# huzi96/gaussian-pcloud-render

Measured on AMD Instinct MI355X. Metric: rendered frames/sec at 1080p (fwd+bwd), THuman-800K, higher is better.
Workload: dtype f32

## Files before the change

gaussian-pcloud-render_amd/csrc/sort.hip:

```cpp
#include "common.hpp"

namespace gsr {

__device__ __forceinline__ uint32_t lane_id() { return __builtin_amdgcn_mbcnt_hi(~0u, __builtin_amdgcn_mbcnt_lo(~0u, 0u)); }

__device__ __forceinline__ uint32_t wave_inclusive_scan(uint32_t v, uint32_t lane)
{
#pragma unroll
    for (int d = 1; d < 64; d <<= 1) {
        const uint32_t n = __shfl_up(v, d, 64);
        if (lane >= (uint32_t)d) v += n;
    }
    return v;
}

__device__ __forceinline__ uint32_t block_exclusive_scan_256(uint32_t v, uint32_t* tmp, uint32_t* total)
{
    const uint32_t lane = threadIdx.x & 63, w = threadIdx.x >> 6;
    const uint32_t inc = wave_inclusive_scan(v, lane);
    if (lane == 63) tmp[w] = inc;
    __syncthreads();
    uint32_t base = 0;
#pragma unroll
    for (int i = 0; i < 4; i++)
        if ((uint32_t)i < w) base += tmp[i];
    if (total) *total = tmp[0] + tmp[1] + tmp[2] + tmp[3];
    __syncthreads();
    return base + inc - v;
}

struct SortView {
    size_t stride;
    const uint64_t* n_dev;
    size_t n_stride;
    int64_t cap;
    const uint32_t* ctl;
};
__device__ __forceinline__ bool pass_control(const SortView& sv, uint32_t view, int shift, uint32_t& base)
{
    base = 0u;
    if (sv.ctl == nullptr) return true;
    const uint32_t* c = at_view(sv.ctl, sv.stride, view);
    base = c[SORTCTL_BASE];
    return (uint32_t)shift < c[SORTCTL_BITS];
}
__device__ __forceinline__ int64_t view_count(const SortView& sv, uint32_t view)
{
    if (sv.n_dev == nullptr) return sv.cap;
    const uint64_t n = *at_view(sv.n_dev, sv.n_stride, view);
    return n < (uint64_t)sv.cap ? (int64_t)n : sv.cap;
}

constexpr int HIST_GROUP = 16;

template <typename KeyT, int RS_ITEMS>
__global__ __launch_bounds__(RS_THREADS) void k_radix_hist(const KeyT* __restrict__ keys, SortView sv, int shift,
                                                           uint32_t mask, uint32_t* __restrict__ hist, int nblk_pad,
                                                           uint32_t* __restrict__ minmax)
{
    constexpr int RS_TILE = RS_THREADS * RS_ITEMS;
    const uint32_t view = blockIdx.y;
    uint32_t kbase;
    if (!pass_control(sv, view, shift, kbase)) return;
    const int64_t n = view_count(sv, view);
    keys = at_view(keys, sv.stride, view);
    hist = at_view(hist, sv.stride, view);
    if (minmax) minmax = at_view(minmax, sv.stride, view);
    const uint32_t d = threadIdx.x;
    if ((int64_t)blockIdx.x * RS_TILE >= n) {
        if (d <= mask) hist[(size_t)d * nblk_pad + blockIdx.x] = 0;
        if (minmax && d == 0) { minmax[blockIdx.x] = 0xFFFFFFFFu; minmax[nblk_pad + blockIdx.x] = 0u; }
        return;
    }
    constexpr int HIST_COPIES = 4 * RS_WAVES;
    __shared__ __attribute__((aligned(16))) uint32_t h[HIST_COPIES][RADIX];
    __shared__ uint32_t s_min, s_max;
    for (int i = threadIdx.x; i < HIST_COPIES * RADIX / 4; i += RS_THREADS) reinterpret_cast<uint4*>(&h[0][0])[i] = make_uint4(0, 0, 0, 0);
    if (threadIdx.x == 0) { s_min = 0xFFFFFFFFu; s_max = 0u; }
    __syncthreads();
    uint32_t kmin = 0xFFFFFFFFu, kmax = 0u;
    const int64_t base = (int64_t)blockIdx.x * RS_TILE;
    const uint32_t w = (threadIdx.x >> 6) * 4u + (threadIdx.x & 3u);
    if (sizeof(KeyT) == 2 && RS_ITEMS % 8 == 0 && base + RS_TILE <= n) {
        const uint4* k4 = reinterpret_cast<const uint4*>(keys + base) + threadIdx.x * (RS_ITEMS / 8);
#pragma unroll
        for (int v = 0; v < RS_ITEMS / 8; v++) {
            const uint4 q = k4[v];
            const uint32_t wds[4] = {q.x, q.y, q.z, q.w};
#pragma unroll
            for (int j = 0; j < 4; j++) {
                atomicAdd(&h[w][((wds[j] & 0xFFFFu) >> shift) & mask], 1u);
                atomicAdd(&h[w][((wds[j] >> 16) >> shift) & mask], 1u);
            }
        }
    } else {
#pragma unroll
        for (int i = 0; i < RS_ITEMS; i++) {
            const int64_t idx = base + i * RS_THREADS + threadIdx.x;
            if (idx < n) {
                const uint32_t key = (uint32_t)keys[idx];
                atomicAdd(&h[w][((key - kbase) >> shift) & mask], 1u);
                if (key != CULLED_KEY) { kmin = key < kmin ? key : kmin; kmax = key > kmax ? key : kmax; }
            }
        }
    }
    if (minmax) {
#pragma unroll
        for (int dd = 32; dd >= 1; dd >>= 1) {
            const uint32_t a = __shfl_xor(kmin, dd, 64), b = __shfl_xor(kmax, dd, 64);
            kmin = a < kmin ? a : kmin;
            kmax = b > kmax ? b : kmax;
        }
        if ((threadIdx.x & 63) == 0) { atomicMin(&s_min, kmin); atomicMax(&s_max, kmax); }
    }
    __syncthreads();
    if (minmax && d == 0) { minmax[blockIdx.x] = s_min; minmax[nblk_pad + blockIdx.x] = s_max; }
    if (d <= mask) {
        uint32_t c = 0;
#pragma unroll
        for (int i = 0; i < HIST_COPIES; i++) c += h[i][d];
        hist[(size_t)d * nblk_pad + blockIdx.x] = c;
    }
}

__global__ __launch_bounds__(256) void k_radix_rowscan(uint32_t* __restrict__ hist, uint32_t* __restrict__ totals, int nblk_pad,
                                                       size_t stride, const uint32_t* __restrict__ ctl, int shift,
                                                       const uint32_t* __restrict__ minmax, uint32_t* __restrict__ ctl_out,
                                                       uint32_t nrows)
{
    __shared__ uint32_t tmp[4];
    if (blockIdx.x == nrows) {
        minmax = at_view(minmax, stride, blockIdx.y);
        uint32_t kmin = 0xFFFFFFFFu, kmax = 0u;
        for (int b = threadIdx.x; b < nblk_pad; b += 256) {
            const uint32_t a = minmax[b], c = minmax[nblk_pad + b];
            kmin = a < kmin ? a : kmin;
            kmax = c > kmax ? c : kmax;
        }
        __shared__ uint32_t s_min, s_max;
        if (threadIdx.x == 0) { s_min = 0xFFFFFFFFu; s_max = 0u; }
        __syncthreads();
        atomicMin(&s_min, kmin);
        atomicMax(&s_max, kmax);
        __syncthreads();
        if (threadIdx.x == 0) {
            uint32_t* c = at_view(ctl_out, stride, blockIdx.y);
            const uint32_t base = s_min <= s_max ? (s_min & ~(uint32_t)(RADIX - 1)) : 0u;
            const uint32_t span = s_min <= s_max ? s_max - base : 0u;
            const uint32_t bits = span ? 32u - (uint32_t)__builtin_clz(span) : 0u;
            c[SORTCTL_BASE] = base;
            c[SORTCTL_BITS] = bits < (uint32_t)RADIX_BITS ? (uint32_t)RADIX_BITS : bits;
        }
        return;
    }
    if (ctl != nullptr && (uint32_t)shift >= at_view(ctl, stride, blockIdx.y)[SORTCTL_BITS]) return;
    hist = at_view(hist, stride, blockIdx.y);
    totals = at_view(totals, stride, blockIdx.y);
    uint32_t* row = hist + (size_t)blockIdx.x * nblk_pad;
    uint32_t carry = 0;
    for (int b0 = 0; b0 < nblk_pad; b0 += 256) {
        const int b = b0 + threadIdx.x;
        const uint32_t v = b < nblk_pad ? row[b] : 0u;
        uint32_t tot;
        const uint32_t ex = block_exclusive_scan_256(v, tmp, &tot);
        if (b < nblk_pad) row[b] = carry + ex;
        carry += tot;
    }
    if (threadIdx.x == 0) totals[blockIdx.x] = carry;
}

#ifdef GSR_STATS
constexpr int SC_REC = 65536;
__device__ unsigned g_sc_rec[SC_REC][5];
#define SC_T(var) const unsigned long long var = wall_clock64()
#define SC_PUT(i, v) do { if (threadIdx.x == 0) { const unsigned r_ = blockIdx.y * gridDim.x + blockIdx.x; if (r_ < SC_REC) g_sc_rec[r_][i] = (unsigned)(v); } } while (0)
int debug_scatter_times(unsigned long long* out8, int reset)
{
    static unsigned host[SC_REC][5];
    if (hipMemcpyFromSymbol(host, HIP_SYMBOL(g_sc_rec), sizeof(host)) != hipSuccess) return -1;
    for (int i = 0; i < 8; i++) out8[i] = 0;
    for (int r = 0; r < SC_REC; r++) {
        if (host[r][1] == 0) continue;
        for (int i = 0; i < 5; i++) out8[i] += host[r][i];
        out8[5]++;
    }
    if (reset) {
        for (int r = 0; r < SC_REC; r++) for (int i = 0; i < 5; i++) host[r][i] = 0;
        if (hipMemcpyToSymbol(HIP_SYMBOL(g_sc_rec), host, sizeof(host)) != hipSuccess) return -1;
    }
    return 0;
}
#else
#define SC_T(var) do { } while (0)
#define SC_PUT(i, v) do { } while (0)
#endif

template <int BITS, typename KeyT, int RS_ITEMS>
__global__ __launch_bounds__(RS_THREADS) void k_radix_scatter(const KeyT* __restrict__ keys_in,
                                                              const uint32_t* __restrict__ vals_in,
                                                              KeyT* __restrict__ keys_out,
                                                              uint32_t* __restrict__ vals_out, SortView sv, int shift,
                                                              uint32_t mask, const uint32_t* __restrict__ hist,
                                                              const uint32_t* __restrict__ totals, int nblk_pad)
{
    constexpr int RS_TILE = RS_THREADS * RS_ITEMS;
    const uint32_t view = blockIdx.y;
    uint32_t kbase;
    if (!pass_control(sv, view, shift, kbase)) return;
    const int64_t n = view_count(sv, view);
    const uint32_t wg = blockIdx.x, xcd = wg & 7u, r = wg >> 3;
    const uint32_t blk = ((r / HIST_GROUP) * 8u + xcd) * HIST_GROUP + (r % HIST_GROUP);
    hist = at_view(hist, sv.stride, view);
    totals = at_view(totals, sv.stride, view);
    if ((int64_t)blk * RS_TILE >= n) return;
    keys_in = at_view(keys_in, sv.stride, view);
    if (vals_in) vals_in = at_view(vals_in, sv.stride, view);
    keys_out = at_view(keys_out, sv.stride, view);
    vals_out = at_view(vals_out, sv.stride, view);
    __shared__ uint32_t s_key[RS_TILE];
    __shared__ uint32_t s_val[RS_TILE];
    __shared__ uint32_t wave_cnt[RS_WAVES][RADIX];
    __shared__ uint32_t local_base[RADIX];
    __shared__ uint32_t global_base[RADIX];
    __shared__ uint32_t tmp[4];

    const uint32_t tid = threadIdx.x, lane = tid & 63, w = tid >> 6;
    const int64_t blk_base = (int64_t)blk * RS_TILE;
    const int64_t seg_base = blk_base + (int64_t)w * (RS_TILE / RS_WAVES);

    for (int i = lane; i < RADIX; i += 64) wave_cnt[w][i] = 0;
    SC_T(t0);

    const uint32_t tot_d = tid <= mask ? totals[tid] : 0u;
    const uint32_t hist_d = tid <= mask ? hist[(size_t)tid * nblk_pad + blk] : 0u;

    uint32_t k[RS_ITEMS], v[RS_ITEMS], rank[RS_ITEMS];
    const bool full = blk_base + RS_TILE <= n;
    {
        const KeyT* kp = keys_in + seg_base + lane;
        const uint32_t* vp = vals_in ? vals_in + seg_base + lane : nullptr;
        if (full) {
#pragma unroll
            for (int j = 0; j < RS_ITEMS; j++) k[j] = (uint32_t)kp[j * 64] - kbase;
            if (vp) {
#pragma unroll
                for (int j = 0; j < RS_ITEMS; j++) v[j] = vp[j * 64];
            } else {
#pragma unroll
                for (int j = 0; j < RS_ITEMS; j++) v[j] = (uint32_t)(seg_base + j * 64 + lane);
            }
        } else {
#pragma unroll
            for (int j = 0; j < RS_ITEMS; j++) {
                const int64_t idx = seg_base + j * 64 + lane;
                const bool ok = idx < n;
                k[j] = ok ? (uint32_t)kp[j * 64] - kbase : 0xFFFFFFFFu;
                v[j] = ok ? (vp ? vp[j * 64] : (uint32_t)idx) : 0u;
            }
        }
    }
    uint32_t gbase_d = block_exclusive_scan_256(tot_d, tmp, nullptr) + hist_d;
    __builtin_amdgcn_wave_barrier();
#ifdef GSR_STATS
    asm volatile("s_waitcnt vmcnt(0)" ::: "memory");
#endif
    SC_T(t1);
    SC_PUT(0, t1 - t0);

#pragma unroll
    for (int j = 0; j < RS_ITEMS; j++) {
        const bool ok = full || seg_base + j * 64 + lane < n;
        const uint32_t d = (k[j] >> shift) & mask;
        const uint64_t okb = full ? ~0ull : __ballot(ok);
        uint32_t plo = (uint32_t)okb, phi = (uint32_t)(okb >> 32);
#pragma unroll
        for (int b = 0; b < BITS; b++) {
            const uint32_t m = (uint32_t)__builtin_amdgcn_sbfe((int32_t)k[j], (uint32_t)(shift + b), 1u);
            const uint64_t bal = __ballot(m != 0u);
            plo = __builtin_amdgcn_bitop3_b32(plo, (uint32_t)bal, m, 0x90);
            phi = __builtin_amdgcn_bitop3_b32(phi, (uint32_t)(bal >> 32), m, 0x90);
        }
        const uint32_t before = wave_cnt[w][d];
        const uint32_t below = __builtin_amdgcn_mbcnt_hi(phi, __builtin_amdgcn_mbcnt_lo(plo, 0u));
        rank[j] = before + below;
        __builtin_amdgcn_wave_barrier();
        if (ok && below == 0) wave_cnt[w][d] = before + (uint32_t)__popc(plo) + (uint32_t)__popc(phi);
        __builtin_amdgcn_wave_barrier();
    }
    __syncthreads();
    SC_T(t2);
    SC_PUT(1, t2 - t1);

    {
        const uint32_t d = tid;
        uint32_t c[RS_WAVES], run = 0;
#pragma unroll
        for (int i = 0; i < RS_WAVES; i++) {
            c[i] = wave_cnt[i][d];
            wave_cnt[i][d] = run;
            run += c[i];
        }
        const uint32_t lbase = block_exclusive_scan_256(run, tmp, nullptr);
        local_base[d] = lbase;
        global_base[d] = gbase_d;
    }
    __syncthreads();
    SC_T(t3);
    SC_PUT(2, t3 - t2);

#pragma unroll
    for (int j = 0; j < RS_ITEMS; j++) {
        if (full || seg_base + j * 64 + lane < n) {
            const uint32_t d = (k[j] >> shift) & mask;
            const uint32_t pos = local_base[d] + wave_cnt[w][d] + rank[j];
            s_key[pos] = k[j];
            s_val[pos] = v[j];
        }
    }
    __syncthreads();
    SC_T(t4);
    SC_PUT(3, t4 - t3);

    const int64_t rem = n - blk_base;
    const uint32_t count = rem < RS_TILE ? (uint32_t)rem : (uint32_t)RS_TILE;
#pragma unroll
    for (int i = 0; i < RS_ITEMS; i++) {
        const uint32_t p = i * RS_THREADS + tid;
        if (p < count) {
            const uint32_t key = s_key[p];
            const uint32_t d = (key >> shift) & mask;
            const size_t g = (size_t)global_base[d] + (p - local_base[d]);
            keys_out[g] = (KeyT)(key + kbase);
            vals_out[g] = s_val[p];
        }
    }
#ifdef GSR_STATS
    { SC_T(t5); SC_PUT(4, t5 - t4); }
#endif
}

int launch_radix_sort_pairs(const Launch& L, const SortJob& job, bool iota_vals, int end_bit, int* result_buffer, bool key16)
{
    int cur = 0;
    if (job.cap > 0 && job.V > 0) {
        const bool small = job.small_blocks && !key16 && end_bit % RADIX_BITS == 0;
        const int tile = small ? RS_TILE_SMALL : RS_TILE;
        const int nblk = (int)div_up(job.cap, tile);
        const int nblk_pad = sort_hist_stride(job.cap, tile);
        SortView sv{job.stride, job.n_dev, job.n_stride, job.cap, nullptr};
        const dim3 grid_hist(nblk_pad, job.V);
        const dim3 grid((unsigned)div_up(nblk, 8 * HIST_GROUP) * 8 * HIST_GROUP, job.V);
        bool first = true;
        const int npass = (end_bit + RADIX_BITS - 1) / RADIX_BITS;
        int shift = 0;
        for (int pass = 0; pass < npass; pass++) {
            const int bits = (end_bit - shift + (npass - pass) - 1) / (npass - pass);
            const uint32_t mask = (1u << bits) - 1u;
            const bool make_ctl = job.sortctl != nullptr && pass == 0;
            sv.ctl = (job.sortctl != nullptr && pass > 0) ? job.sortctl : nullptr;
            uint32_t* minmax = make_ctl ? job.blk_minmax : nullptr;
            if (key16)
                hipLaunchKernelGGL((k_radix_hist<uint16_t, RS_ITEMS>), grid_hist, dim3(RS_THREADS), 0, L.stream, (const uint16_t*)job.key[cur], sv,
                                   shift, mask, job.hist, nblk_pad, minmax);
            else if (small)
                hipLaunchKernelGGL((k_radix_hist<uint32_t, RS_ITEMS_SMALL>), grid_hist, dim3(RS_THREADS), 0, L.stream, (const uint32_t*)job.key[cur], sv,
                                   shift, mask, job.hist, nblk_pad, minmax);
            else
                hipLaunchKernelGGL((k_radix_hist<uint32_t, RS_ITEMS>), grid_hist, dim3(RS_THREADS), 0, L.stream, (const uint32_t*)job.key[cur], sv,
                                   shift, mask, job.hist, nblk_pad, minmax);
            if (int e = check_launch(L, "radix_hist")) return e;
            hipLaunchKernelGGL(k_radix_rowscan, dim3(mask + 1u + (make_ctl ? 1u : 0u), job.V), dim3(256), 0, L.stream, job.hist,
                               job.totals, nblk_pad, job.stride, sv.ctl, shift, (const uint32_t*)minmax, job.sortctl, mask + 1u);
            if (int e = check_launch(L, "radix_rowscan")) return e;
            const uint32_t* vin = (first && iota_vals) ? (const uint32_t*)nullptr : (const uint32_t*)job.val[cur];
#define GSR_SCATTER(B)                                                                                                        \
    case B:                                                                                                                   \
        if (key16)                                                                                                            \
            hipLaunchKernelGGL((k_radix_scatter<B, uint16_t, RS_ITEMS>), grid, dim3(RS_THREADS), 0, L.stream,                 \
                               (const uint16_t*)job.key[cur], vin, (uint16_t*)job.key[cur ^ 1], job.val[cur ^ 1], sv, shift,  \
                               mask, job.hist, job.totals, nblk_pad);                                                         \
        else                                                                                                                  \
            hipLaunchKernelGGL((k_radix_scatter<B, uint32_t, RS_ITEMS>), grid, dim3(RS_THREADS), 0, L.stream,                 \
                               (const uint32_t*)job.key[cur], vin, job.key[cur ^ 1], job.val[cur ^ 1], sv, shift, mask,       \
                               job.hist, job.totals, nblk_pad);                                                               \
        break;
            if (small)
                hipLaunchKernelGGL((k_radix_scatter<RADIX_BITS, uint32_t, RS_ITEMS_SMALL>), grid, dim3(RS_THREADS), 0, L.stream,
                                   (const uint32_t*)job.key[cur], vin, job.key[cur ^ 1], job.val[cur ^ 1], sv, shift, mask, job.hist,
                                   job.totals, nblk_pad);
            else switch (bits) {
                GSR_SCATTER(1) GSR_SCATTER(2) GSR_SCATTER(3) GSR_SCATTER(4) GSR_SCATTER(5) GSR_SCATTER(6) GSR_SCATTER(7)
                GSR_SCATTER(8)
            }
#undef GSR_SCATTER
            if (int e = check_launch(L, "radix_scatter")) return e;
            cur ^= 1;
            first = false;
            shift += bits;
        }
    } else {
        cur = ((end_bit + RADIX_BITS - 1) / RADIX_BITS) & 1;
    }
    *result_buffer = cur;
    return GSR_OK;
}

}
```

Before: 2153.

## Restructure radix histogram: digit-major copies sized by pass bits, coalesced prefetch

Reworks the radix histogram kernel so the shared-memory histogram is digit-major, with the number of per-thread copies scaled to the pass's digit count (template NB chosen from bits). Keys for full tiles are now loaded with coalesced 16-byte strided loads issued before the shared-memory clear, and the 32-bit key path also uses vector loads. The final reduction reads four uint4s per thread and combines them with a wave shuffle. The aim is fewer atomic conflicts and cheaper reductions on narrow passes, and overlap of global loads with shared init. The cost is more template instantiations and added register pressure from holding keys in registers.

```diff
diff --git a/gaussian-pcloud-render_amd/csrc/sort.hip b/gaussian-pcloud-render_amd/csrc/sort.hip
--- a/gaussian-pcloud-render_amd/csrc/sort.hip
+++ b/gaussian-pcloud-render_amd/csrc/sort.hip
@@ -52,13 +52,19 @@
 }
 
 constexpr int HIST_GROUP = 16;
-
-template <typename KeyT, int RS_ITEMS>
+constexpr int HIST_WORDS = 4 * RS_WAVES * RADIX;
+
+template <typename KeyT, int RS_ITEMS, int NB>
 __global__ __launch_bounds__(RS_THREADS) void k_radix_hist(const KeyT* __restrict__ keys, SortView sv, int shift,
                                                            uint32_t mask, uint32_t* __restrict__ hist, int nblk_pad,
                                                            uint32_t* __restrict__ minmax)
 {
     constexpr int RS_TILE = RS_THREADS * RS_ITEMS;
+    constexpr int NV = RS_ITEMS * (int)sizeof(KeyT) / 16;
+    static_assert(NV >= 1 && NV * 16 == RS_ITEMS * (int)sizeof(KeyT), "a thread's keys of a full block are whole 16-B loads");
+    constexpr uint32_t COPIES = HIST_WORDS / NB;
+    constexpr uint32_t GROUPS = RS_THREADS / NB;
+    static_assert((NB == 64 || NB == 128 || NB == 256) && COPIES == 16 * GROUPS, "a thread sums 16 words");
     const uint32_t view = blockIdx.y;
     uint32_t kbase;
     if (!pass_control(sv, view, shift, kbase)) return;
@@ -72,25 +78,36 @@
         if (minmax && d == 0) { minmax[blockIdx.x] = 0xFFFFFFFFu; minmax[nblk_pad + blockIdx.x] = 0u; }
         return;
     }
-    constexpr int HIST_COPIES = 4 * RS_WAVES;
-    __shared__ __attribute__((aligned(16))) uint32_t h[HIST_COPIES][RADIX];
+    const int64_t base = (int64_t)blockIdx.x * RS_TILE;
+    const bool full = base + RS_TILE <= n;
+    uint4 q[NV];
+    if (full) {
+        const uint4* k4 = reinterpret_cast<const uint4*>(keys + base) + threadIdx.x;
+#pragma unroll
+        for (int v = 0; v < NV; v++) q[v] = k4[v * RS_THREADS];
+    }
+    __shared__ __attribute__((aligned(16))) uint32_t h[HIST_WORDS];
     __shared__ uint32_t s_min, s_max;
-    for (int i = threadIdx.x; i < HIST_COPIES * RADIX / 4; i += RS_THREADS) reinterpret_cast<uint4*>(&h[0][0])[i] = make_uint4(0, 0, 0, 0);
+    for (int i = threadIdx.x; i < HIST_WORDS / 4; i += RS_THREADS) reinterpret_cast<uint4*>(h)[i] = make_uint4(0, 0, 0, 0);
     if (threadIdx.x == 0) { s_min = 0xFFFFFFFFu; s_max = 0u; }
     __syncthreads();
     uint32_t kmin = 0xFFFFFFFFu, kmax = 0u;
-    const int64_t base = (int64_t)blockIdx.x * RS_TILE;
-    const uint32_t w = (threadIdx.x >> 6) * 4u + (threadIdx.x & 3u);
-    if (sizeof(KeyT) == 2 && RS_ITEMS % 8 == 0 && base + RS_TILE <= n) {
-        const uint4* k4 = reinterpret_cast<const uint4*>(keys + base) + threadIdx.x * (RS_ITEMS / 8);
-#pragma unroll
-        for (int v = 0; v < RS_ITEMS / 8; v++) {
-            const uint4 q = k4[v];
-            const uint32_t wds[4] = {q.x, q.y, q.z, q.w};
+    const uint32_t copy = threadIdx.x & (COPIES - 1u);
+    const auto count = [&](uint32_t digit) { atomicAdd(&h[digit * COPIES + copy], 1u); };
+    if (full) {
+#pragma unroll
+        for (int v = 0; v < NV; v++) {
+            const uint32_t wds[4] = {q[v].x, q[v].y, q[v].z, q[v].w};
 #pragma unroll
             for (int j = 0; j < 4; j++) {
-                atomicAdd(&h[w][((wds[j] & 0xFFFFu) >> shift) & mask], 1u);
-                atomicAdd(&h[w][((wds[j] >> 16) >> shift) & mask], 1u);
+                if (sizeof(KeyT) == 2) {
+                    count(((wds[j] & 0xFFFFu) >> shift) & mask);
+                    count(((wds[j] >> 16) >> shift) & mask);
+                } else {
+                    const uint32_t key = wds[j];
+                    count(((key - kbase) >> shift) & mask);
+                    if (key != CULLED_KEY) { kmin = key < kmin ? key : kmin; kmax = key > kmax ? key : kmax; }
+                }
             }
         }
     } else {
@@ -99,7 +116,7 @@
             const int64_t idx = base + i * RS_THREADS + threadIdx.x;
             if (idx < n) {
                 const uint32_t key = (uint32_t)keys[idx];
-                atomicAdd(&h[w][((key - kbase) >> shift) & mask], 1u);
+                count(((key - kbase) >> shift) & mask);
                 if (key != CULLED_KEY) { kmin = key < kmin ? key : kmin; kmax = key > kmax ? key : kmax; }
             }
         }
@@ -115,12 +132,16 @@
     }
     __syncthreads();
     if (minmax && d == 0) { minmax[blockIdx.x] = s_min; minmax[nblk_pad + blockIdx.x] = s_max; }
-    if (d <= mask) {
-        uint32_t c = 0;
-#pragma unroll
-        for (int i = 0; i < HIST_COPIES; i++) c += h[i][d];
-        hist[(size_t)d * nblk_pad + blockIdx.x] = c;
-    }
+    uint32_t c = 0;
+#pragma unroll
+    for (int i = 0; i < 4; i++) {
+        const uint4 x = reinterpret_cast<const uint4*>(h)[d * 4 + i];
+        c += x.x + x.y + x.z + x.w;
+    }
+#pragma unroll
+    for (uint32_t x = 1; x < GROUPS; x <<= 1) c += __shfl_xor(c, x, 64);
+    const uint32_t digit = d / GROUPS;
+    if ((d & (GROUPS - 1u)) == 0 && digit <= mask) hist[(size_t)digit * nblk_pad + blockIdx.x] = c;
 }
 
 __global__ __launch_bounds__(256) void k_radix_rowscan(uint32_t* __restrict__ hist, uint32_t* __restrict__ totals, int nblk_pad,
@@ -359,15 +380,16 @@
             const bool make_ctl = job.sortctl != nullptr && pass == 0;
             sv.ctl = (job.sortctl != nullptr && pass > 0) ? job.sortctl : nullptr;
             uint32_t* minmax = make_ctl ? job.blk_minmax : nullptr;
-            if (key16)
-                hipLaunchKernelGGL((k_radix_hist<uint16_t, RS_ITEMS>), grid_hist, dim3(RS_THREADS), 0, L.stream, (const uint16_t*)job.key[cur], sv,
-                                   shift, mask, job.hist, nblk_pad, minmax);
-            else if (small)
-                hipLaunchKernelGGL((k_radix_hist<uint32_t, RS_ITEMS_SMALL>), grid_hist, dim3(RS_THREADS), 0, L.stream, (const uint32_t*)job.key[cur], sv,
-                                   shift, mask, job.hist, nblk_pad, minmax);
-            else
-                hipLaunchKernelGGL((k_radix_hist<uint32_t, RS_ITEMS>), grid_hist, dim3(RS_THREADS), 0, L.stream, (const uint32_t*)job.key[cur], sv,
-                                   shift, mask, job.hist, nblk_pad, minmax);
+#define GSR_HIST(KT, ITEMS, NB)                                                                                               \
+    hipLaunchKernelGGL((k_radix_hist<KT, ITEMS, NB>), grid_hist, dim3(RS_THREADS), 0, L.stream, (const KT*)job.key[cur], sv, shift, mask, \
+                       job.hist, nblk_pad, minmax)
+#define GSR_HIST_NB(KT, ITEMS)                                                                                                \
+    do { if (bits <= 6) GSR_HIST(KT, ITEMS, 64); else if (bits == 7) GSR_HIST(KT, ITEMS, 128); else GSR_HIST(KT, ITEMS, 256); } while (0)
+            if (key16) GSR_HIST_NB(uint16_t, RS_ITEMS);
+            else if (small) GSR_HIST_NB(uint32_t, RS_ITEMS_SMALL);
+            else GSR_HIST_NB(uint32_t, RS_ITEMS);
+#undef GSR_HIST_NB
+#undef GSR_HIST
             if (int e = check_launch(L, "radix_hist")) return e;
             hipLaunchKernelGGL(k_radix_rowscan, dim3(mask + 1u + (make_ctl ? 1u : 0u), job.V), dim3(256), 0, L.stream, job.hist,
                                job.totals, nblk_pad, job.stride, sv.ctl, shift, (const uint32_t*)minmax, job.sortctl, mask + 1u);
```

New measurement: 2174 (median of 6 runs). Within noise of the previous version (+0.9%).
